# dotchen/LAV

Hardware: AMD Instinct MI355X
Metric: frames/s full agent fwd (32k-pt LiDAR + 3 cams) (higher is better)
Workload: dtype f32 (convolution contractions on the matrix cores with f32 accumulate at the error of an fp32 dot product, DESIGN 4.3: the layers on the split-operand kernel - BEV backbone, heads, crop stems, the brake net's mid-size layers - and ERFNet's persistent runs of pairs as two power-of-two-scaled fp16 pie

## Files before the change

### include/lav_amd.h

```cpp
#ifndef LAV_AMD_H
#define LAV_AMD_H

#include <stddef.h>
#include <stdint.h>

#ifdef __cplusplus
extern "C" {
#endif

#define LAV_ABI_VERSION 40

#define LAV_OK 0
#define LAV_EINVAL (-1)
#define LAV_EHIP (-2)
#define LAV_EWORKSPACE (-3)

int lav_abi_version(void);
const char *lav_last_error(void);
int lav_device_count(void);

int lav_profile_enable(int slots);
int lav_profile_reset(void);
int lav_profile_read(const char *kernel, double *total_ms, int *launches);

typedef struct lav_grid {
    float min_x, max_x, min_y, max_y;
    float ppm;
    int nx, ny;
} lav_grid;

typedef struct lav_pointnet {
    const float *w1, *b1, *w2, *b2;
    int num_input;
    int channels;
} lav_pointnet;

size_t lav_pillar_workspace_bytes(int batch, int max_points, const lav_grid *grid);
int lav_pillar_workspace_init(void *workspace, size_t workspace_bytes, void *stream);

int lav_pillar_scatter(const float *points, const int *h_num_points, int batch, int max_points, int D,
                       const lav_grid *grid, const lav_pointnet *net, float *canvas,
                       int *unique_coords, int *inverse, int *counts,
                       void *workspace, size_t workspace_bytes, void *stream);
// ... 180 lines not shown
int lav_upconv_pointwise_parts(int batch, int cin, int cout, int ih, int iw, int k, int pad, int out_pad);
int lav_upconv_pointwise(int batch, int cin, int cout, int ih, int iw, int k, int pad, int out_pad, const float *x, const float *w_packed,
                         const float *scale, const float *shift, int relu_pre, int out_c_total, int out_c_offset, float *y,
                         float *amax_out, void *stream);

size_t lav_conv1d_pair_packed_weight_floats(int channels);
int lav_conv1d_pair_pack_weights(int channels, const float *h_weight, float *h_packed);
size_t lav_conv1d_pair_chain_workspace_bytes(int batch, int h);
size_t lav_conv1d_pair_chain_lds_bytes(int channels, int w, int d_b_max);
int lav_conv1d_pair_chain(int batch, int channels, int h, int w, int npairs, const int *d_a, const int *d_b, const int *residual,
                          const int *relu_post, const float *x, const float *const *wa_packed, const float *const *bias_a,
                          const float *const *wb_packed, const float *const *bias_b, const float *const *scale,
                          const float *const *shift, float *const *out, void *workspace, size_t workspace_bytes, void *stream);
int lav_conv1d_pair_chain_f16(int batch, int channels, int h, int w, int npairs, const int *d_a, const int *d_b, const int *residual,
                              const int *relu_post, const float *x, const float *const *wa_packed, const float *const *bias_a,
                              const float *const *wb_packed, const float *const *bias_b, const float *const *scale,
                              const float *const *shift, float *const *out, void *workspace, size_t workspace_bytes, void *stream);
int lav_conv1d_pair_chain_region(int row_offset, int clean_rows);
int lav_conv1d_pair_chain_status(const void *workspace, int *h_timeouts_launches2, void *stream);
size_t lav_conv1d_pair_lds_bytes(int channels, int w, int d_b);
size_t lav_conv3x3_run_f16_workspace_bytes(int channels, int h, int w, int nlayers);
size_t lav_conv3x3_run_f16_lds_bytes(int channels, int h, int w);
size_t lav_conv3x3_run_f16_weight_bytes(int channels);
int lav_conv3x3_run_f16_amax_count(int channels, int h, int w);
long lav_conv_f16_weights_offset(const lav_conv *c);
int lav_conv3x3_run_f16(int channels, int h, int w, int nlayers, const float *x, const void *const *w_f16, const float *const *scale,
                        const float *const *shift, float *out, const float *amax_in, int amax_in_count, float *amax_out, void *workspace,
                        size_t workspace_bytes, void *stream);
int lav_conv3x3_run_f16_status(const void *workspace, int *h_timeouts_launches2, void *stream);
size_t lav_conv3x3_tile_f16_lds_bytes(int channels, int h, int w, int nlayers);
int lav_conv3x3_tile_f16_amax_count(int channels, int h, int w, int nlayers);
int lav_conv3x3_tile_f16(int channels, int h, int w, int nlayers, const float *x, const void *const *w_f16, const float *const *scale,
                         const float *const *shift, float *out, const float *amax_in, int amax_in_count, float *amax_out, void *stream);
int lav_conv1d_pair(int batch, int channels, int h, int w, int d_a, int d_b, const float *x, const float *wa_packed,
                    const float *bias_a, const float *wb_packed, const float *bias_b, const float *scale, const float *shift,
                    const float *residual, int relu_post, float *y, void *stream);

int lav_pool_affine(const float *x, int batch, int channels, int h, int w, const float *scale, const float *shift, int relu,
                    float *y, int out_c_total, int out_c_offset, void *stream);

int lav_pair_train_supported(int channels, int width);
size_t lav_pair_train_workspace_bytes(int batch, int channels, int h);
int lav_pair_train_forward(const float *x, const float *wa, const float *ba, const float *wb, const float *bb, int batch, int channels,
                           int h, int w, int dil, float *t, float *z, void *stream);
int lav_pair_train_backward(const float *x, const float *t, const float *dz, const float *wa, const float *wb, int batch, int channels,
                            int h, int w, int dil, float *dt, float *dx, float *dwa, float *dba, float *dwb, float *dbb, void *workspace,
                            size_t workspace_bytes, void *stream);

size_t lav_seg_xent_workspace_bytes(void);
int lav_seg_xent_forward(const float *logits, const long long *labels, int batch, int classes, long plane, float *loss, float *dlogits,
                         void *workspace, size_t workspace_bytes, void *stream);

int lav_seg_xent_up_forward(const float *logits, const void *labels, int label_bytes, int batch, int classes, int h, int w, int scale,
                            float *loss, float *dlogits, void *workspace, size_t workspace_bytes, void *stream);

typedef struct lav_camera_f64 {
    double l2w[16];
    double w2c[16];
    double K[9];
} lav_camera_f64;

int lav_paint_frames(const float *lidar, const int *offsets, int frames, int total, int lidar_dim, const float *sem, int ncam,
                     int sem_c, int h, int w, const lav_camera_f64 *h_cams, float *painted, int *uvz, void *stream);

int lav_image_u8_to_f32(const unsigned char *img, int n, int h, int w, int c_src, int reverse, float *out, void *stream);

// ... 59 lines not shown
```

### lav_amd/_lib.py

```python
from __future__ import annotations

import ctypes as C
import os

HERE = os.path.dirname(os.path.abspath(__file__))
LIB_PATH = os.environ.get("LAV_AMD_LIB") or os.path.join(HERE, "liblav_amd.so")

ABI_VERSION = 40
MAX_CAM = 4
MAX_CAM_F64 = 8


class Grid(C.Structure):
    _fields_ = [("min_x", C.c_float), ("max_x", C.c_float), ("min_y", C.c_float), ("max_y", C.c_float),
                ("ppm", C.c_float), ("nx", C.c_int), ("ny", C.c_int)]


class PointNet(C.Structure):
    _fields_ = [("w1", C.c_void_p), ("b1", C.c_void_p), ("w2", C.c_void_p), ("b2", C.c_void_p),
                ("num_input", C.c_int), ("channels", C.c_int)]


class Camera(C.Structure):
    _fields_ = [("K", C.c_float * 9), ("l2w", C.c_float * 16), ("w2c", C.c_float * 16)]


class CameraF64(C.Structure):
    _fields_ = [("l2w", C.c_double * 16), ("w2c", C.c_double * 16), ("K", C.c_double * 9)]


class Conv(C.Structure):
    _fields_ = [(n, C.c_int) for n in (
        "batch", "in_c_total", "in_c_offset", "cin", "h", "w", "cout", "kh", "kw", "stride", "pad_h", "pad_w",
        "dil_h", "dil_w", "transposed", "out_pad", "out_c_total", "out_c_offset", "relu_pre", "relu_post", "sigmoid", "target_cus")] + [("pad_value", C.c_float), ("precision", C.c_int)]


CONV_F32, CONV_BF16X6, CONV_F16X3 = 1, 2, 3


_P, _I, _Z, _F = C.c_void_p, C.c_int, C.c_size_t, C.c_float
SIGNATURES = {
# ... 28 lines not shown
    "lav_conv_pack_map_ints": (_Z, [C.POINTER(Conv)]),
    "lav_conv_pack_map": (_I, [C.POINTER(Conv), _P]),
    "lav_conv_repack": (_I, [C.POINTER(Conv), _P, _P, _P, _P]),
    "lav_conv_repack_scratch": (_I, [C.POINTER(Conv), _P, _P, _P, _P, _Z, _P]),
    "lav_bn_fold": (_I, [_P, _P, _P, _P, C.c_double, _I, _P, _P, _P]),
    "lav_conv_wgrad_workspace_bytes": (_Z, [_I, _I, _I, _I, _I, _I, _I]),
    "lav_conv_wgrad": (_I, [_P, _P, _I, _I, _I, _I, _I, _I, _I, _P, _P, _Z, _P]),
    "lav_conv_wgrad_amax": (_I, [_P, _P, _I, _I, _I, _I, _I, _I, _I, _P, _P, _Z, _P, _I, _P, _I, _P]),
    "lav_absmax_parts": (_I, [_P, C.c_long, _P, _P]),
    "lav_conv_tile_info": (_I, [C.POINTER(Conv), C.POINTER(_I)]),
    "lav_conv_workspace_bytes": (_Z, [C.POINTER(Conv)]),
    "lav_conv2d": (_I, [C.POINTER(Conv), _P, _P, _P, _P, _P, _P, _P, _P, _Z, _P]),
    "lav_conv_amax_count": (_I, [C.POINTER(Conv)]),
    "lav_conv2d_amax": (_I, [C.POINTER(Conv), _P, _P, _P, _P, _P, _P, _P, _P, _Z, _P, _I, _P, _P]),
    "lav_deconv_grouped": (_I, [_I, _I, _I, _I, _I, C.POINTER(_I), _I, _I, _I, _I, _P, _P, _P, _I, _P, _P]),
    "lav_crop_rotate": (_I, [_P, _I, _I, _I, _I, _P, _P, _I, _F, _I, _F, _F, _P, _P]),
    "lav_crop_rotate_indexed": (_I, [_P, _I, _P, _I, _I, _I, _P, _P, _I, _F, _I, _F, _F, _P, _P]),
    "lav_crop_rotate_backward": (_I, [_P, _I, _P, _I, _I, _I, _P, _P, _I, _F, _I, _F, _F, _P, _P]),
    "lav_pillar_decorate": (_I, [_P, C.POINTER(_I), _I, _I, _I, C.POINTER(Grid), _P, _P, _P, _P, _P, _P, _Z, _P]),
    "lav_scatter_max": (_I, [_P, _P, _I, _I, _I, _P, _P, _P]),
    "lav_scatter_max_backward": (_I, [_P, _P, _I, _I, _I, _P, _P]),
    "lav_conv1d_pair_packed_weight_floats": (_Z, [_I]),
    "lav_conv1d_pair_pack_weights": (_I, [_I, _P, _P]),
    "lav_upconv_pointwise_packed_floats": (_Z, [_I, _I, _I]),
    "lav_upconv_pointwise_pack": (_I, [_I, _I, _I, _P, _P]),
    "lav_upconv_pointwise_parts": (_I, [_I] * 8),
    "lav_upconv_pointwise": (_I, [_I] * 8 + [_P, _P, _P, _P, _I, _I, _I, _P, _P, _P]),
    "lav_conv1d_pair_chain_workspace_bytes": (_Z, [_I, _I]),
    "lav_conv1d_pair_chain_region": (_I, [_I, _I]),
    "lav_conv1d_pair_chain_lds_bytes": (_Z, [_I, _I, _I]),
    "lav_conv1d_pair_chain": (_I, [_I, _I, _I, _I, _I, C.POINTER(_I), C.POINTER(_I), C.POINTER(_I), C.POINTER(_I), _P] + [C.POINTER(_P)] * 7 + [_P, _Z, _P]),
    "lav_conv1d_pair_chain_f16": (_I, [_I, _I, _I, _I, _I, C.POINTER(_I), C.POINTER(_I), C.POINTER(_I), C.POINTER(_I), _P] + [C.POINTER(_P)] * 7 + [_P, _Z, _P]),
    "lav_conv1d_pair_chain_status": (_I, [_P, C.POINTER(_I), _P]),
    "lav_conv1d_pair_lds_bytes": (_Z, [_I, _I, _I]),
    "lav_conv3x3_run_f16_workspace_bytes": (_Z, [_I, _I, _I, _I]),
    "lav_conv3x3_run_f16_lds_bytes": (_Z, [_I, _I, _I]),
    "lav_conv3x3_run_f16_weight_bytes": (_Z, [_I]),
    "lav_conv3x3_run_f16_amax_count": (_I, [_I, _I, _I]),
    "lav_conv_f16_weights_offset": (C.c_long, [C.POINTER(Conv)]),
    "lav_conv3x3_run_f16": (_I, [_I, _I, _I, _I, _P, C.POINTER(_P), C.POINTER(_P), C.POINTER(_P), _P, _P, _I, _P, _P, _Z, _P]),
    "lav_conv3x3_run_f16_status": (_I, [_P, C.POINTER(_I), _P]),
    "lav_conv3x3_tile_f16_lds_bytes": (_Z, [_I, _I, _I, _I]),
    "lav_conv3x3_tile_f16_amax_count": (_I, [_I, _I, _I, _I]),
    "lav_conv3x3_tile_f16": (_I, [_I, _I, _I, _I, _P, C.POINTER(_P), C.POINTER(_P), C.POINTER(_P), _P, _P, _I, _P, _P]),
    "lav_conv1d_pair": (_I, [_I, _I, _I, _I, _I, _I, _P, _P, _P, _P, _P, _P, _P, _P, _I, _P, _P]),
    "lav_gru_seq_forward": (_I, [_P, _I, _P, _P, _P, _I, _I, _I, _P, _P, _P]),
    "lav_gru_seq_backward_workspace_bytes": (_Z, [_I, _I]),
    "lav_gru_seq_backward": (_I, [_P, _P, _P, _P, _P, _I, _I, _I, _P, _P, _P, _P, _Z, _P]),
    "lav_bn_train_workspace_bytes": (_Z, [_I]),
    "lav_bn_train_forward_mask": (_I, [_P, _P, _P, _P, _I, _I, C.c_long, _P, _P, C.c_double, _I, _P, _P, _P, _P, _P, _Z, _P]),
    "lav_bn_train_backward_mask": (_I, [_P, _P, _P, _P, _I, _I, C.c_long, _P, _P, _P, _I, _P, _P, _P, _P, _P, _P, _Z, _P]),
    "lav_pair_train_supported": (_I, [_I, _I]),
    "lav_pair_train_workspace_bytes": (_Z, [_I, _I, _I]),
    "lav_pair_train_forward": (_I, [_P, _P, _P, _P, _P, _I, _I, _I, _I, _I, _P, _P, _P]),
    "lav_pair_train_backward": (_I, [_P, _P, _P, _P, _P, _I, _I, _I, _I, _I, _P, _P, _P, _P, _P, _P, _P, _Z, _P]),
    "lav_seg_xent_workspace_bytes": (_Z, []),
    "lav_seg_xent_forward": (_I, [_P, _P, _I, _I, C.c_long, _P, _P, _P, _Z, _P]),
    "lav_seg_xent_up_forward": (_I, [_P, _P, _I, _I, _I, _I, _I, _I, _P, _P, _P, _Z, _P]),
    "lav_attn_train_workspace_bytes": (_Z, [_I, _I, _I, _I]),
    "lav_attn_train_forward": (_I, [_P, _I, _I, _I, _I, _P, _P, _P, _P, C.c_float, _P, _P, _P, _P, _P, _P]),
    "lav_attn_train_backward": (_I, [_P, _I, _I, _I, _I, _P, _P, _P, _P, C.c_float, _P, _P, _P, _P, _P, _P, _P, _P, _P, _Z, _P]),
    "lav_bn_train_forward": (_I, [_P, _P, _P, _I, _I, C.c_long, _P, _P, C.c_double, _I, _I, _P, _P, _P, _P, _Z, _P]),
    "lav_bn_train_backward": (_I, [_P, _P, _P, _I, _I, C.c_long, _P, _P, _P, _I, _I, _P, _P, _P, _P, _P, _Z, _P]),
    "lav_bn_train_amax_count": (_I, [_I, _I, C.c_long]),
    "lav_bn_train_forward_amax": (_I, [_P, _P, _P, _I, _I, C.c_long, _P, _P, C.c_double, _I, _I, _P, _P, _P, _P, _P, _Z, _P]),
    "lav_bn_train_backward_amax": (_I, [_P, _P, _P, _I, _I, C.c_long, _P, _P, _P, _I, _I, _P, _P, _P, _P, _P, _P, _Z, _P]),
# ... 66 lines not shown
```

### lav_amd/build.py

```python
from __future__ import annotations

import os
import subprocess
import sys
import time

HERE = os.path.dirname(os.path.abspath(__file__))
REPO = os.path.dirname(HERE)
CSRC = os.path.join(HERE, "csrc")
LIB = os.path.join(HERE, "liblav_amd.so")
SOURCES = ["misc.hip", "pillar.hip", "paint.hip", "paint_frames.hip", "gru.hip", "gru_seq.hip", "conv.hip", "conv_f16.hip", "conv_pair.hip", "conv_run.hip", "conv_tile.hip", "deconv.hip", "crop.hip", "frame.hip", "attn.hip", "bn_train.hip", "conv_wgrad.hip", "upconv.hip", "conv_pair_train.hip", "augment.hip", "bev_stack.hip", "debug_view.hip", "log_view.hip", "eval_metrics.hip", "eval_camera.hip", "eval_plans.hip"]
EXTRA_FLAGS = {"pillar.hip": ["-ffp-contract=off"], "paint.hip": ["-ffp-contract=off"], "paint_frames.hip": ["-ffp-contract=off"], "crop.hip": ["-ffp-contract=off"],
               "frame.hip": ["-ffp-contract=off"], "augment.hip": ["-ffp-contract=off"], "bev_stack.hip": ["-ffp-contract=off"],
               "debug_view.hip": ["-ffp-contract=off", "-fhip-fp32-correctly-rounded-divide-sqrt"],
               "log_view.hip": ["-ffp-contract=off"],
               "eval_metrics.hip": ["-ffp-contract=off"],
               "eval_plans.hip": ["-ffp-contract=off"]}
FLAGS = ["--offload-arch=gfx950", "-O3", "-std=c++17", "-fPIC", "-Wall", "-Wno-unused-function", "-fno-slp-vectorize",
         "-I", os.path.join(REPO, "include"), "-I", CSRC]


def _hipcc() -> str:
    for c in (os.environ.get("HIPCC"), "/opt/rocm/bin/hipcc", "hipcc"):
        if c and (os.path.isabs(c) and os.path.exists(c) or not os.path.isabs(c)):
            return c
    raise RuntimeError("hipcc not found")


def needs_build() -> bool:
    if not os.path.exists(LIB):
        return True
    t = os.path.getmtime(LIB)
    deps = [os.path.join(CSRC, f) for f in os.listdir(CSRC)] + [os.path.join(REPO, "include", "lav_amd.h")]
    return any(os.path.getmtime(d) > t for d in deps)


def build(force: bool = False, verbose: bool = True) -> str:
    if not force and not needs_build():
        return LIB
    objs = []
    procs = []
    os.makedirs(os.path.join(HERE, "build"), exist_ok=True)
    t0 = time.time()
    for s in SOURCES:
# ... 22 lines not shown
```

### lav_amd/erfnet.py

```python
from __future__ import annotations

import os

import torch
import torch.nn as nn
import torch.nn.functional as F

from . import ops
from .ops import Conv1dPair, Conv1dPairChain, ConvLayer, GroupedDeconv, infer_precision

_USE_PAIRS = os.environ.get("LAV_ERFNET_PAIRS", "1") != "0"


def _affine(bn, sl):
    s = (bn.weight.detach().double() / torch.sqrt(bn.running_var.detach().double() + bn.eps))
    t = bn.bias.detach().double() - bn.running_mean.detach().double() * s
    return s[sl].float()[None, :, None, None].contiguous(), t[sl].float()[None, :, None, None].contiguous()


class DownsamplerBlock(nn.Module):
    def __init__(self, cin, cout):
        super().__init__()
        self.conv = nn.Conv2d(cin, cout - cin, 3, stride=2, padding=1, bias=True)
        self.pool = nn.MaxPool2d(2, stride=2)
        self.bn = nn.BatchNorm2d(cout, eps=1e-3)

    def forward(self, x):
        return F.relu(self.bn(torch.cat([self.conv(x), self.pool(x)], 1)))

    def engine(self, device, input_affine=None):
        from . import ops
        nconv = self.conv.out_channels
        cout = self.bn.num_features
        w, b, pad = self.conv.weight.detach(), self.conv.bias.detach(), 0.0
        s_in, t_in = (1.0, 0.0) if input_affine is None else input_affine
        if input_affine is not None:
            if not s_in > 0:
                raise RuntimeError("input_affine needs a positive scale")
            b = (b.double() + t_in * w.double().sum(dim=(1, 2, 3))).float()
            w = (w.double() * s_in).float()
            pad = -t_in / s_in
        sl = slice(0, nconv)
# ... 34 lines not shown
        if self.dropout.p != 0:
            y = self.dropout(y)
        return F.relu(y + x)

    def engine(self, device):
        a = ConvLayer.from_module(self.conv3x1_1, relu_post=True, device=device)
        b = ConvLayer.from_module(self.conv1x3_1, self.bn1, relu_post=True, device=device)
        c = ConvLayer.from_module(self.conv3x1_2, relu_post=True, device=device)
        d = ConvLayer.from_module(self.conv1x3_2, self.bn2, relu_post=True, device=device)
        p1 = Conv1dPair(self.conv3x1_1, self.conv1x3_1, self.bn1, device=device)
        p2 = Conv1dPair(self.conv3x1_2, self.conv1x3_2, self.bn2, device=device)

        def run(x):
            if _USE_PAIRS and p1.supported(x) and p2.supported(x):
                return p2(p1(x), residual=x)
            return d(c(b(a(x))), residual=x)
        run.pairs = (p1, p2)
        return run


def _chain_blocks(stages):
    out, run = [], []

    def flush():
        if not run:
            return
        blocks = list(run)
        run.clear()
        if len(blocks) == 1 or not _USE_PAIRS:
            out.extend(blocks)
            return
        pairs = [p for b in blocks for p in b.pairs]
        chain = Conv1dPairChain(pairs, [i % 2 == 1 for i in range(len(pairs))])

        def go(x):
            if chain.supported(x):
                return chain(x)
            for b in blocks:
                x = b(x)
            return x
        go.chain = chain
        out.append(go)

    for st in stages:
        if getattr(st, "pairs", None) is not None and (not run or run[-1].pairs[0].ch == st.pairs[0].ch):
            run.append(st)
        else:
            flush()
            if getattr(st, "pairs", None) is not None:
                run.append(st)
            else:
                out.append(st)
    flush()
    return out


class UpsamplerBlock(nn.Module):
    def __init__(self, cin, cout):
        super().__init__()
        self.conv = nn.ConvTranspose2d(cin, cout, 3, stride=2, padding=1, output_padding=1, bias=True)
        self.bn = nn.BatchNorm2d(cout, eps=1e-3)

    def forward(self, x):
        return F.relu(self.bn(self.conv(x)))

    def engine(self, device):
        return ConvLayer.from_module(self.conv, self.bn, relu_post=True, device=device)


class Encoder(nn.Module):
    def __init__(self, num_classes):
        super().__init__()
        self.initial_block = DownsamplerBlock(3, 16)
        blocks = [DownsamplerBlock(16, 64)] + [non_bottleneck_1d(64, 0.03, 1) for _ in range(5)] + [DownsamplerBlock(64, 128)]
# ... 14 lines not shown
        self.layers = nn.ModuleList([UpsamplerBlock(128, 64), non_bottleneck_1d(64, 0, 1), non_bottleneck_1d(64, 0, 1),
                                     UpsamplerBlock(64, 16), non_bottleneck_1d(16, 0, 1), non_bottleneck_1d(16, 0, 1)])
        self.output_conv = nn.ConvTranspose2d(16, num_classes, 2, stride=2)

    def forward(self, x):
        for layer in self.layers:
            x = layer(x)
        return self.output_conv(x)


class ERFNet(nn.Module):
    def __init__(self, num_classes):
        super().__init__()
        self.encoder = Encoder(num_classes)
        self.decoder = Decoder(num_classes)
        object.__setattr__(self, "_eng", None)

    def _drop(self):
        object.__setattr__(self, "_eng", None)

    def _apply(self, fn, *a, **k):
        self._drop()
        return super()._apply(fn, *a, **k)

    def train(self, mode: bool = True):
        self._drop()
        return super().train(mode)

    def _load_from_state_dict(self, *a, **k):
        self._drop()
        return super()._load_from_state_dict(*a, **k)

    def _engine(self, device, input_affine=None, softmax=False):
        key = (device, input_affine, softmax, infer_precision())
        if self._eng is None or self._eng[0] != key:
            stages = [self.encoder.initial_block.engine(device, input_affine)]
            stages += [m.engine(device) for m in self.encoder.layers]
            stages += [m.engine(device) for m in self.decoder.layers]
            stages = _chain_blocks(stages)
            stages.append(GroupedDeconv([self.decoder.output_conv], softmax=softmax, device=device))
            object.__setattr__(self, "_eng", (key, stages))
        return self._eng[1]

    def forward(self, x, input_affine=None, softmax=False):
        if self.training:
            if input_affine is not None:
                x = x * input_affine[0] + input_affine[1]
            y = self.decoder(self.encoder(x))
            return torch.softmax(y, dim=1) if softmax else y
        if not x.is_cuda:
            raise RuntimeError("ERFNet: eval-mode forward needs a tensor in HBM - lav_amd has no CPU path "
                               "(CPU evaluation for tests and baselines: oracle/camera.py)")
        shared = os.environ.get("LAV_CHAIN_SHARED_CLEAN", "1") != "0"
        cap, off, first = ops.pair_chain_capacity(x.device), 0, True
        for stage in self._engine(x.device, input_affine, softmax):
            chain = getattr(stage, "chain", None)
            rows = x.shape[0] * x.shape[2]
            if shared and chain is not None and chain.supported(x) and off + rows <= cap:
                with ops.pair_chain_region(off, cap if first else 0):
                    x = stage(x)
                off, first = off + rows, False
            else:
                if chain is not None:
                    shared = False
                x = stage(x)
        return x
```

### lav_amd/ops.py

```python
from __future__ import annotations

import ctypes as C
import os as _os
import threading as _threading
from typing import Optional, Sequence

import numpy as np
import torch

from . import _lib
from ._lib import Camera, Conv, Grid, PointNet, check

_workspaces: dict = {}


def _stream() -> int:
    return torch.cuda.current_stream().cuda_stream


def _ptr(t: Optional[torch.Tensor]) -> Optional[int]:
    return None if t is None else t.data_ptr()


def _f32c(t: torch.Tensor, name: str) -> torch.Tensor:
# ... 1029 lines not shown


class Conv1dPairChain:

    def __init__(self, pairs, residual):
        if len(pairs) != len(residual) or not pairs or residual[0]:
            raise RuntimeError("Conv1dPairChain: one residual flag per pair, the first pair without")
        if any(p.ch != pairs[0].ch or p.scale is None for p in pairs):
            raise RuntimeError("Conv1dPairChain: pairs of one channel count, each with its BatchNorm affine")
        self.pairs, self.residual = list(pairs), [int(bool(r)) for r in residual]
        self._bufs = {}
        self.f16 = infer_precision() == _lib.CONV_F16X3 and _os.environ.get("LAV_ERFNET_F16", "1") != "0"

    def supported(self, x: torch.Tensor) -> bool:
        lib = _lib.load()
        B, ch, h, w = x.shape
        p0 = self.pairs[0]
        lds = lib.lav_conv1d_pair_chain_lds_bytes(p0.ch, w, max(p.db for p in self.pairs))
        return (_os.environ.get("LAV_CONV_PRECISION", "bf16x6") not in ("f32", "fp32") and _os.environ.get("LAV_ERFNET_CHAIN", "1") != "0"
                and len(self.pairs) <= 16 and all(p.supported(x) for p in self.pairs)
                and B * h <= _cu_count(x.device) * (2 if (lds <= 76 * 1024 and not (ch >= 64 and (ch // 16) % 2 == 0)) else 1)
                and lds <= 152 * 1024)

    def __call__(self, x: torch.Tensor) -> torch.Tensor:
        lib = _lib.load()
        x = _f32c(x, "x")
        B, ch, h, w = x.shape
        n = len(self.pairs)
        key = (B, h, w, x.device, _stream())
        bufs = self._bufs.get(key)
        if bufs is None:
            bufs = self._bufs[key] = [torch.empty_like(x) for _ in range(n - 1)]
        out = bufs + [torch.empty_like(x)]
        ws = _workspace("pair_chain", max(lib.lav_conv1d_pair_chain_workspace_bytes(B, h), lib.lav_conv1d_pair_chain_workspace_bytes(pair_chain_capacity(x.device), 1)), x.device)
        ia = lambda vals: (C.c_int * n)(*vals)
        pa = lambda ts: (C.c_void_p * n)(*[t.data_ptr() for t in ts])
        ps = self.pairs
        check((lib.lav_conv1d_pair_chain_f16 if self.f16 else lib.lav_conv1d_pair_chain)(B, ch, h, w, n, ia([p.da for p in ps]), ia([p.db for p in ps]), ia(self.residual),
                                        ia([int(p.relu_post) for p in ps]), _ptr(x), pa([p.wa for p in ps]), pa([p.ba for p in ps]),
                                        pa([p.wb for p in ps]), pa([p.bb for p in ps]), pa([p.scale for p in ps]), pa([p.shift for p in ps]),
                                        pa(out), _ptr(ws), ws.numel(), _stream()), "lav_conv1d_pair_chain")
        return out[-1]

    def timeouts(self, x_like: torch.Tensor) -> int:
        return pair_chain_status(x_like.device)[0]


def pair_chain_capacity(device) -> int:
    return 4 * _cu_count(device)


class pair_chain_region:

    def __init__(self, row_offset: int, clean_rows: int):
        self.args = (int(row_offset), int(clean_rows))

    def __enter__(self):
        check(_lib.load().lav_conv1d_pair_chain_region(*self.args), "lav_conv1d_pair_chain_region")
        return self

    def __exit__(self, *exc):
        check(_lib.load().lav_conv1d_pair_chain_region(0, -1), "lav_conv1d_pair_chain_region")
        return False


def pair_chain_status(device, stream=None):
    st = stream if stream is not None else torch.cuda.current_stream()
    device = torch.device(device)
    if device.index is None:
        device = torch.device("cuda", torch.cuda.current_device())
    ws = _workspaces.get(("pair_chain", device, st.cuda_stream))
    if ws is None:
        return (0, 0)
    v = (C.c_int * 2)()
    check(_lib.load().lav_conv1d_pair_chain_status(_ptr(ws), v, st.cuda_stream), "lav_conv1d_pair_chain_status")
    return (int(v[0]), int(v[1]))


def bev_run_stages():
    v = _os.environ.get("LAV_BEV_RUN", BEV_RUN_DEFAULT).strip().lower()
    if v in ("0", "", "off", "none"):
        return frozenset()
    if v in ("1", "on", "all"):
        return frozenset(("s1", "s2", "s3"))
    return frozenset(s for s in v.split(",") if s in ("s1", "s2", "s3"))


BEV_RUN_DEFAULT = "s2,s3"


class ConvRun:

    def __init__(self, layers):
        lib = _lib.load()
        layers = list(layers)
        l0 = layers[0]
        for l in layers:
            d = l.desc
            if not (d.precision == _lib.CONV_F16X3 and (d.kh, d.kw, d.stride, d.pad_h, d.pad_w, d.dil_h, d.dil_w) == (3, 3, 1, 1, 1, 1, 1)
                    and not d.transposed and l.cin == l.cout == l0.cin and l.in_c_total == l.cin and l.out_c_total == l.cout
                    and l.bias is None and l.scale is not None and d.relu_pre and not d.relu_post and not d.sigmoid and d.pad_value == 0.0):
                raise RuntimeError("ConvRun: layers must be identical conv3x3 / ReLU / BatchNorm layers packed for LAV_CONV_F16X3")
        self.layers, self.ch = layers, l0.cin
        probe = Conv.from_buffer_copy(l0.desc)
        probe.h, probe.w = 64, 64
        self._woff = int(lib.lav_conv_f16_weights_offset(C.byref(probe)))
        if self._woff < 0 or len(layers) > 8:
            raise RuntimeError("ConvRun: at most 8 layers with fp16 packed weights")
        n = len(layers)
# ... 324 lines not shown
```

Measured before the change: 541.0.

## Add spatially tiled fused non-bottleneck-1d kernel for ERFNet dilation-1 blocks

Adds a new kernel that runs one or two whole ERFNet non-bottleneck-1d blocks (four 1D convolution pairs with BN, ReLU and residual) inside a single workgroup per spatial tile. Activations stay in LDS as split fp16 pieces with a halo, and the next layer's weights are prefetched into registers while the current layer runs. The goal is to avoid the global round-trips and row-wise chain scheduling of the existing pair-chain path. By default it is enabled only for the 16-channel, two-block stage, at the cost of recomputing halo regions and a large LDS footprint.

```diff
diff --git a/include/lav_amd.h b/include/lav_amd.h
--- a/include/lav_amd.h
+++ b/include/lav_amd.h
@@ -8,7 +8,7 @@
 extern "C" {
 #endif
 
-#define LAV_ABI_VERSION 40
+#define LAV_ABI_VERSION 41
 
 #define LAV_OK 0
 #define LAV_EINVAL (-1)
@@ -255,6 +255,10 @@
 int lav_conv3x3_tile_f16_amax_count(int channels, int h, int w, int nlayers);
 int lav_conv3x3_tile_f16(int channels, int h, int w, int nlayers, const float *x, const void *const *w_f16, const float *const *scale,
                          const float *const *shift, float *out, const float *amax_in, int amax_in_count, float *amax_out, void *stream);
+size_t lav_nb1d_tile_f16_lds_bytes(int channels, int h, int w, int nblocks);
+int lav_nb1d_tile_f16(int batch, int channels, int h, int w, int nblocks, const float *x, const float *const *wa_packed,
+                      const float *const *bias_a, const float *const *wb_packed, const float *const *bias_b, const float *const *scale,
+                      const float *const *shift, float *out, void *count_workspace, void *stream);
 int lav_conv1d_pair(int batch, int channels, int h, int w, int d_a, int d_b, const float *x, const float *wa_packed,
                     const float *bias_a, const float *wb_packed, const float *bias_b, const float *scale, const float *shift,
                     const float *residual, int relu_post, float *y, void *stream);
diff --git a/lav_amd/_lib.py b/lav_amd/_lib.py
--- a/lav_amd/_lib.py
+++ b/lav_amd/_lib.py
@@ -6,7 +6,7 @@
 HERE = os.path.dirname(os.path.abspath(__file__))
 LIB_PATH = os.environ.get("LAV_AMD_LIB") or os.path.join(HERE, "liblav_amd.so")
 
-ABI_VERSION = 40
+ABI_VERSION = 41
 MAX_CAM = 4
 MAX_CAM_F64 = 8
 
@@ -101,6 +101,8 @@
     "lav_conv1d_pair_chain": (_I, [_I, _I, _I, _I, _I, C.POINTER(_I), C.POINTER(_I), C.POINTER(_I), C.POINTER(_I), _P] + [C.POINTER(_P)] * 7 + [_P, _Z, _P]),
     "lav_conv1d_pair_chain_f16": (_I, [_I, _I, _I, _I, _I, C.POINTER(_I), C.POINTER(_I), C.POINTER(_I), C.POINTER(_I), _P] + [C.POINTER(_P)] * 7 + [_P, _Z, _P]),
     "lav_conv1d_pair_chain_status": (_I, [_P, C.POINTER(_I), _P]),
+    "lav_nb1d_tile_f16_lds_bytes": (_Z, [_I, _I, _I, _I]),
+    "lav_nb1d_tile_f16": (_I, [_I, _I, _I, _I, _I, _P] + [C.POINTER(_P)] * 6 + [_P, _P, _P]),
     "lav_conv1d_pair_lds_bytes": (_Z, [_I, _I, _I]),
     "lav_conv3x3_run_f16_workspace_bytes": (_Z, [_I, _I, _I, _I]),
     "lav_conv3x3_run_f16_lds_bytes": (_Z, [_I, _I, _I]),
diff --git a/lav_amd/build.py b/lav_amd/build.py
--- a/lav_amd/build.py
+++ b/lav_amd/build.py
@@ -9,7 +9,7 @@
 REPO = os.path.dirname(HERE)
 CSRC = os.path.join(HERE, "csrc")
 LIB = os.path.join(HERE, "liblav_amd.so")
-SOURCES = ["misc.hip", "pillar.hip", "paint.hip", "paint_frames.hip", "gru.hip", "gru_seq.hip", "conv.hip", "conv_f16.hip", "conv_pair.hip", "conv_run.hip", "conv_tile.hip", "deconv.hip", "crop.hip", "frame.hip", "attn.hip", "bn_train.hip", "conv_wgrad.hip", "upconv.hip", "conv_pair_train.hip", "augment.hip", "bev_stack.hip", "debug_view.hip", "log_view.hip", "eval_metrics.hip", "eval_camera.hip", "eval_plans.hip"]
+SOURCES = ["misc.hip", "pillar.hip", "paint.hip", "paint_frames.hip", "gru.hip", "gru_seq.hip", "conv.hip", "conv_f16.hip", "conv_pair.hip", "conv_pair_tile.hip", "conv_run.hip", "conv_tile.hip", "deconv.hip", "crop.hip", "frame.hip", "attn.hip", "bn_train.hip", "conv_wgrad.hip", "upconv.hip", "conv_pair_train.hip", "augment.hip", "bev_stack.hip", "debug_view.hip", "log_view.hip", "eval_metrics.hip", "eval_camera.hip", "eval_plans.hip"]
 EXTRA_FLAGS = {"pillar.hip": ["-ffp-contract=off"], "paint.hip": ["-ffp-contract=off"], "paint_frames.hip": ["-ffp-contract=off"], "crop.hip": ["-ffp-contract=off"],
                "frame.hip": ["-ffp-contract=off"], "augment.hip": ["-ffp-contract=off"], "bev_stack.hip": ["-ffp-contract=off"],
                "debug_view.hip": ["-ffp-contract=off", "-fhip-fp32-correctly-rounded-divide-sqrt"],
diff --git a/lav_amd/csrc/conv_pair_tile.hip b/lav_amd/csrc/conv_pair_tile.hip
--- /dev/null
+++ b/lav_amd/csrc/conv_pair_tile.hip
@@ -0,0 +1,424 @@
+#include <cstdlib>
+#include <cstring>
+
+#include "common.hpp"
+#include "split_arith.hpp"
+
+namespace {
+using namespace lav;
+
+constexpr int NBT_MAX_NB = 2, NBT_MAX_PAIRS = 2 * NBT_MAX_NB;
+
+struct NbTileArgs {
+    const float *x;
+    float *out;
+    const unsigned char *wA[NBT_MAX_PAIRS], *wB[NBT_MAX_PAIRS];
+    const float *tA[NBT_MAX_PAIRS], *tB[NBT_MAX_PAIRS];
+    const float *bA[NBT_MAX_PAIRS], *bB[NBT_MAX_PAIRS], *scale[NBT_MAX_PAIRS], *shift[NBT_MAX_PAIRS];
+    int *count;
+    int H, W, tiles_x, tiles_y;
+};
+
+template <int C>
+struct NbGeo {
+    static constexpr int NCH = C / 16, CBLK = (C + 31) / 32, NGRP = 8 / CBLK, NG8 = C / 8;
+    static constexpr int NPART = C >= 64 ? 2 : 1;
+    static constexpr int NGV = C >= 32 ? 4 : C / 8;
+    static constexpr int WB = 3 * NCH * CBLK * 2 * 1024;
+    static constexpr int NPF = (WB / 16 + 511) / 512;
+};
+
+template <int C>
+__device__ __forceinline__ void nbt_w_fetch(const unsigned char *w, u32x4 (&pf)[NbGeo<C>::NPF]) {
+#pragma unroll
+    for (int k = 0; k < NbGeo<C>::NPF; ++k) {
+        const int u = threadIdx.x + 512 * k;
+        pf[k] = *reinterpret_cast<const u32x4 *>(w + min(u, NbGeo<C>::WB / 16 - 1) * 16);
+    }
+}
+template <int C>
+__device__ __forceinline__ void nbt_w_store(unsigned char *wl, const u32x4 (&pf)[NbGeo<C>::NPF]) {
+#pragma unroll
+    for (int k = 0; k < NbGeo<C>::NPF; ++k) {
+        const int u = threadIdx.x + 512 * k;
+        if (u < NbGeo<C>::WB / 16) *reinterpret_cast<u32x4 *>(wl + u * 16) = pf[k];
+    }
+}
+
+template <int C, int NA, int MAXJ, bool VERT, int IW, int NPI>
+__device__ __forceinline__ void nbt_mma(const unsigned char *in, const int (&base)[MAXJ], int half, const unsigned char *wl, f32x16 (&tot)[MAXJ]) {
+    using G = NbGeo<C>;
+    constexpr int PIECE = G::NG8 * NPI * 16, CPP = G::NCH / G::NPART;
+#pragma unroll
+    for (int part = 0; part < G::NPART; ++part) {
+        f32x16 acc[NA];
+#pragma unroll
+        for (int j = 0; j < NA; ++j)
+#pragma unroll
+            for (int r = 0; r < 16; ++r) acc[j][r] = 0.f;
+#pragma unroll
+        for (int i = 0; i < CPP; ++i) {
+            const int ch = part * CPP + i;
+            const unsigned char *bin = in + (ch * 2 + half) * NPI * 16;
+#pragma unroll
+            for (int t = 0; t < 3; ++t) {
+                const int toff = (VERT ? t * IW : t) * 16;
+                u32x4 b[NA][2], wf[2];
+                wf[0] = *reinterpret_cast<const u32x4 *>(wl + (t * G::NCH + ch) * G::CBLK * 2048);
+                wf[1] = *reinterpret_cast<const u32x4 *>(wl + (t * G::NCH + ch) * G::CBLK * 2048 + 1024);
+#pragma unroll
+                for (int j = 0; j < NA; ++j) {
+                    b[j][0] = *reinterpret_cast<const u32x4 *>(bin + toff + base[j]);
+                    b[j][1] = *reinterpret_cast<const u32x4 *>(bin + PIECE + toff + base[j]);
+                }
+#pragma unroll
+                for (int k = 0; k < 3; ++k)
+#pragma unroll
+                    for (int j = 0; j < NA; ++j)
+                        acc[j] = __builtin_amdgcn_mfma_f32_32x32x16_f16(__builtin_bit_cast(f16x8, wf[F16X3_A[k]]), __builtin_bit_cast(f16x8, b[j][F16X3_B[k]]),
+                                                                        acc[j], 0, 0, 0);
+            }
+        }
+#pragma unroll
+        for (int j = 0; j < NA; ++j) {
+            if (part == 0) tot[j] = acc[j];
+            else
+#pragma unroll
+                for (int r = 0; r < 16; ++r) tot[j][r] += acc[j][r];
+        }
+    }
+}
+
+enum { NBT_MID = 0,
+       NBT_PAIR = 1,
+       NBT_BLOCK = 2,
+       NBT_LAST = 3 };
+
+struct NbtScale { float s, m; };
+
+template <int C, int TH, int TW, int IH, int IW, bool VERT, int KIND, bool RES_LDS>
+__device__ __forceinline__ NbtScale nbt_layer(const NbTileArgs &a, int n, int ty0, int tx0, const unsigned char *in, unsigned char *outb, float *res, int iy0, int ix0,
+                                              NbtScale sc, float sw, float l1, float bmax, const float *epi, float *s_wmax, unsigned char *wlds,
+                                              const unsigned char *w_next) {
+    using G = NbGeo<C>;
+    constexpr int OH = VERT ? IH - 2 : IH, OW = VERT ? IW : IW - 2, NP = OH * OW, NPI = IH * IW;
+    constexpr int NBLK = (NP + 31) / 32, MAXJ = (NBLK + G::NGRP - 1) / G::NGRP;
+    const int tid = threadIdx.x, lane = tid & 63, l31 = lane & 31, half = lane >> 5;
+    const int wid = __builtin_amdgcn_readfirstlane(tid >> 6);
+    const int cbw = wid % G::CBLK, grp = wid / G::CBLK;
+    const int H = a.H, W = a.W;
+    const long plane = (long)H * W;
+    const int oy0 = VERT ? iy0 + 1 : iy0, ox0 = VERT ? ix0 : ix0 + 1;
+
+    int qu[MAXJ], base[MAXJ];
+#pragma unroll
+    for (int j = 0; j < MAXJ; ++j) {
+        qu[j] = (grp + G::NGRP * j) * 32 + l31;
+        const int q = min(qu[j], NP - 1);
+        base[j] = ((q / OW) * IW + (q % OW)) * 16;
+    }
+    const int nact = (NBLK - grp + G::NGRP - 1) / G::NGRP;
+
+    float rin[(KIND >= NBT_BLOCK && !RES_LDS) ? MAXJ : 1][16];
+    if constexpr (KIND >= NBT_BLOCK && !RES_LDS) {
+#pragma unroll
+        for (int j = 0; j < MAXJ; ++j) {
+            const int q = min(qu[j], NP - 1);
+            const int gy = oy0 + q / OW, gx = ox0 + q % OW;
+            const bool ok = j < nact && gy >= 0 && gy < H && gx >= 0 && gx < W;
+            const float *xr = a.x + (long)n * C * plane + (long)min(max(gy, 0), H - 1) * W + min(max(gx, 0), W - 1);
+#pragma unroll
+            for (int r = 0; r < 16; ++r) {
+                const int co = min(cbw * 32 + (r & 3) + 8 * (r >> 2) + 4 * half, C - 1);
+                rin[j][r] = ok ? xr[co * plane] : 0.f;
+            }
+        }
+    }
+
+    u32x4 pf[G::NPF];
+    if constexpr (KIND != NBT_LAST) nbt_w_fetch<C>(w_next, pf);
+    f32x16 acc[MAXJ];
+#pragma unroll
+    for (int j = 0; j < MAXJ; ++j)
+#pragma unroll
+        for (int r = 0; r < 16; ++r) acc[j][r] = 0.f;
+    const unsigned char *wl = wlds + cbw * 2048 + lane * 16;
+    if (nact == MAXJ) nbt_mma<C, MAXJ, MAXJ, VERT, IW, NPI>(in, base, half, wl, acc);
+    else if constexpr (MAXJ > 1) nbt_mma<C, MAXJ - 1, MAXJ, VERT, IW, NPI>(in, base, half, wl, acc);
+    if constexpr (KIND == NBT_MID) __syncthreads();
+
+    NbtScale so;
+    float f_in, inv_out = 0.f;
+    if constexpr (KIND == NBT_MID) {
+        so.m = fminf(fmaf(sc.m, l1, bmax), 3.0e38f);
+        so.s = f16_scale_of(so.m);
+        inv_out = 1.f / so.s;
+    }
+    f_in = sc.s * sw;
+    float lm = 0.f;
+    bool inmap[MAXJ];
+#pragma unroll
+    for (int j = 0; j < MAXJ; ++j) {
+        const int q = min(qu[j], NP - 1);
+        const int qy = q / OW, qx = q % OW, gy = oy0 + qy, gx = ox0 + qx;
+        inmap[j] = j < nact && qu[j] < NP && gy >= 0 && gy < H && gx >= 0 && gx < W;
+        float *yo = a.out + (long)n * C * plane + (long)gy * W + gx;
+#pragma unroll
+        for (int r = 0; r < 16; ++r) {
+            if ((r >> 2) >= G::NGV) { acc[j][r] = 0.f; continue; }
+            const int co = cbw * 32 + (r & 3) + 8 * (r >> 2) + 4 * half;
+            float vv;
+            if constexpr (KIND == NBT_MID) {
+                vv = fmaf(acc[j][r], f_in, epi[co]);
+                vv = vv > 0.f ? vv : 0.f;
+            } else {
+                vv = fmaf(fmaf(acc[j][r], f_in, epi[C + co]), epi[2 * C + co], epi[3 * C + co]);
+                if constexpr (KIND >= NBT_BLOCK) {
+                    if constexpr (RES_LDS) vv += inmap[j] ? res[co * (TH * TW) + q] : 0.f;
+                    else vv += rin[j][r];
+                }
+                vv = vv > 0.f ? vv : 0.f;
+            }
+            vv = inmap[j] ? vv : 0.f;
+            if constexpr (KIND == NBT_LAST) {
+                if (inmap[j]) yo[co * plane] = vv;
+            } else {
+                acc[j][r] = vv;
+                lm = fmaxf(lm, finite_abs(vv));
+            }
+            if constexpr (KIND == NBT_BLOCK) {
+                const int ry = qy - 2, rx = qx - 2;
+                if (j < nact && qu[j] < NP && ry >= 0 && ry < TH && rx >= 0 && rx < TW) res[co * (TH * TW) + ry * TW + rx] = vv;
+            }
+        }
+    }
+    if constexpr (KIND == NBT_LAST) return NbtScale{0.f, 0.f};
+    if constexpr (KIND != NBT_MID) {
+        lm = wave_finite_absmax(lm);
+        if (lane == 0) s_wmax[wid] = lm;
+        __syncthreads();
+        float m = 0.f;
+#pragma unroll
+        for (int i = 0; i < 8; ++i) m = fmaxf(m, s_wmax[i]);
+        so.m = m;
+        so.s = f16_scale_of(m);
+        inv_out = 1.f / so.s;
+    }
+#pragma unroll
+    for (int j = 0; j < MAXJ; ++j) {
+        if (j < nact && qu[j] < NP) {
+#pragma unroll
+            for (int g = 0; g < G::NGV; ++g) {
+                unsigned p00, p01, p10, p11;
+                split2h_pair(acc[j][4 * g] * inv_out, acc[j][4 * g + 1] * inv_out, p00, p10);
+                split2h_pair(acc[j][4 * g + 2] * inv_out, acc[j][4 * g + 3] * inv_out, p01, p11);
+                unsigned char *d = outb + ((cbw * 4 + g) * NP + qu[j]) * 16 + half * 8;
+                *reinterpret_cast<u32x2 *>(d) = u32x2{p00, p01};
+                lds_store_fence();
+                *reinterpret_cast<u32x2 *>(d + G::NG8 * NP * 16) = u32x2{p10, p11};
+                lds_store_fence();
+            }
+        }
+    }
+    nbt_w_store<C>(wlds, pf);
+    __syncthreads();
+    return so;
+}
+
+template <int C, int TH, int TW, int NB>
+struct NbTileLds {
+    static constexpr int RH = TH + 4 * NB, RW = TW + 4 * NB;
+    static constexpr int BUF_A = 2 * (C / 8) * RH * RW * 16, BUF_B = 2 * (C / 8) * (RH - 2) * RW * 16;
+    static constexpr int RES = NB > 1 ? TH * TW * C * 4 : 0, EPI = 2 * NB * 4 * C * 4, WB = NbGeo<C>::WB;
+    static constexpr int TOTAL = BUF_A + BUF_B + RES + WB + EPI + 64;
+};
+
+template <int C, int TH, int TW, int IH, int IW, bool LAST, bool RES_LDS>
+__device__ __forceinline__ NbtScale nbt_block(const NbTileArgs &a, int n, int ty0, int tx0, unsigned char *bufA, unsigned char *bufB, float *res, int iy0, int ix0,
+                                              NbtScale sc, int p0, const float (&bmax)[NBT_MAX_PAIRS], const float (&tl)[NBT_MAX_PAIRS][3], const float *s_epi, float *s_wmax,
+                                              unsigned char *wr, const unsigned char *w_after) {
+    const float *e0 = s_epi + p0 * 4 * C, *e1 = e0 + 4 * C;
+    NbtScale s = nbt_layer<C, TH, TW, IH, IW, true, NBT_MID, false>(a, n, ty0, tx0, bufA, bufB, res, iy0, ix0, sc, tl[p0][0], tl[p0][1], bmax[p0], e0, s_wmax, wr,
+                                                                    a.wB[p0]);
+    s = nbt_layer<C, TH, TW, IH - 2, IW, false, NBT_PAIR, false>(a, n, ty0, tx0, bufB, bufA, res, iy0 + 1, ix0, s, tl[p0][2], 0.f, 0.f, e0, s_wmax, wr, a.wA[p0 + 1]);
+    s = nbt_layer<C, TH, TW, IH - 2, IW - 2, true, NBT_MID, false>(a, n, ty0, tx0, bufA, bufB, res, iy0 + 1, ix0 + 1, s, tl[p0 + 1][0], tl[p0 + 1][1], bmax[p0 + 1], e1,
+                                                                   s_wmax, wr, a.wB[p0 + 1]);
+    return nbt_layer<C, TH, TW, IH - 4, IW - 2, false, LAST ? NBT_LAST : NBT_BLOCK, RES_LDS>(a, n, ty0, tx0, bufB, bufA, res, iy0 + 2, ix0 + 1, s, tl[p0 + 1][2], 0.f, 0.f,
+                                                                                            e1, s_wmax, wr, w_after);
+}
+
+template <int C, int TH, int TW, int NB>
+__global__ __launch_bounds__(512) void k_nb1d_tile_f16(NbTileArgs a) {
+    using G = NbGeo<C>;
+    using L = NbTileLds<C, TH, TW, NB>;
+    extern __shared__ __attribute__((aligned(16))) unsigned char smem[];
+    constexpr int RH = L::RH, RW = L::RW, NPA = RH * RW, HALO = 2 * NB;
+    unsigned char *bufA = smem, *bufB = smem + L::BUF_A;
+    float *res = reinterpret_cast<float *>(smem + L::BUF_A + L::BUF_B);
+    unsigned char *wr = smem + L::BUF_A + L::BUF_B + L::RES;
+    float *s_epi = reinterpret_cast<float *>(smem + L::BUF_A + L::BUF_B + L::RES + L::WB);
+    float *s_wmax = s_epi + 2 * NB * 4 * C;
+    const int tid = threadIdx.x, lane = tid & 63;
+    const int wid = __builtin_amdgcn_readfirstlane(tid >> 6);
+    const int H = a.H, W = a.W;
+    const long plane = (long)H * W;
+    const int tiles = a.tiles_x * a.tiles_y;
+    const int n = blockIdx.x / tiles, t_ = blockIdx.x - n * tiles;
+    const int ty0 = (t_ / a.tiles_x) * TH, tx0 = (t_ % a.tiles_x) * TW;
+    if (blockIdx.x == 0 && tid == 0 && a.count) atomicAdd(a.count, 1);
+
+    NbtScale sc;
+    float bmax[NBT_MAX_PAIRS], tails[NBT_MAX_PAIRS][3];
+    {
+        constexpr int NTASK = NPA * G::NG8, NTK = (NTASK + 511) / 512, NEPI = 2 * NB * 4 * C;
+        static_assert(NEPI <= 512, "one epilogue value per thread");
+        float v[NTK][8];
+        bool ok[NTK];
+#pragma unroll
+        for (int u = 0; u < NTK; ++u) {
+            const int task = min(tid + u * 512, NTASK - 1);
+            const int g = task / NPA, p = task - g * NPA;
+            const int gy = ty0 - HALO + p / RW, gx = tx0 - HALO + p % RW;
+            ok[u] = gy >= 0 && gy < H && gx >= 0 && gx < W;
+            const float *sp = a.x + ((long)n * C + g * 8) * plane + (long)min(max(gy, 0), H - 1) * W + min(max(gx, 0), W - 1);
+#pragma unroll
+            for (int c = 0; c < 8; ++c) v[u][c] = sp[c * plane];
+        }
+        u32x4 pf[G::NPF];
+        nbt_w_fetch<C>(a.wA[0], pf);
+        float ev, braw[NBT_MAX_PAIRS];
+        {
+            const int i = min(tid, NEPI - 1), p = i / (4 * C), k = (i / C) & 3, c = i % C;
+            ev = (k == 0 ? a.bA[p] : k == 1 ? a.bB[p] : k == 2 ? a.scale[p] : a.shift[p])[c];
+        }
+#pragma unroll
+        for (int p = 0; p < NBT_MAX_PAIRS; ++p) {
+            braw[p] = a.bA[p][min(lane, C - 1)];
+            tails[p][0] = a.tA[p][0]; tails[p][1] = a.tA[p][1]; tails[p][2] = a.tB[p][0];
+        }
+        float lm = 0.f;
+#pragma unroll
+        for (int u = 0; u < NTK; ++u)
+#pragma unroll
+            for (int c = 0; c < 8; ++c) {
+                v[u][c] = ok[u] ? v[u][c] : 0.f;
+                lm = fmaxf(lm, finite_abs(v[u][c]));
+            }
+        nbt_w_store<C>(wr, pf);
+        if (tid < NEPI) s_epi[tid] = ev;
+#pragma unroll
+        for (int p = 0; p < NBT_MAX_PAIRS; ++p) bmax[p] = wave_finite_absmax(finite_abs(braw[p]));
+        lm = wave_finite_absmax(lm);
+        if (lane == 0) s_wmax[wid] = lm;
+        __syncthreads();
+        float m = 0.f;
+#pragma unroll
+        for (int i = 0; i < 8; ++i) m = fmaxf(m, s_wmax[i]);
+        sc.m = m;
+        sc.s = f16_scale_of(m);
+        const float inv = 1.f / sc.s;
+#pragma unroll
+        for (int u = 0; u < NTK; ++u) {
+            const int task = tid + u * 512;
+            if (task < NTASK) {
+                u32x4 q0, q1;
+#pragma unroll
+                for (int e = 0; e < 4; ++e) {
+                    unsigned p0, p1;
+                    split2h_pair(v[u][2 * e] * inv, v[u][2 * e + 1] * inv, p0, p1);
+                    q0[e] = p0; q1[e] = p1;
+                }
+                *reinterpret_cast<u32x4 *>(bufA + task * 16) = q0;
+                *reinterpret_cast<u32x4 *>(bufA + L::BUF_A / 2 + task * 16) = q1;
+            }
+        }
+    }
+    __syncthreads();
+
+    if constexpr (NB == 1) {
+        nbt_block<C, TH, TW, RH, RW, true, false>(a, n, ty0, tx0, bufA, bufB, res, ty0 - 2, tx0 - 2, sc, 0, bmax, tails, s_epi, s_wmax, wr, nullptr);
+    } else {
+        sc = nbt_block<C, TH, TW, RH, RW, false, false>(a, n, ty0, tx0, bufA, bufB, res, ty0 - 4, tx0 - 4, sc, 0, bmax, tails, s_epi, s_wmax, wr, a.wA[2]);
+        nbt_block<C, TH, TW, RH - 4, RW - 4, true, true>(a, n, ty0, tx0, bufA, bufB, res, ty0 - 2, tx0 - 2, sc, 2, bmax, tails, s_epi, s_wmax, wr, nullptr);
+    }
+}
+
+struct NbTileConfig { int th, tw, tiles_x, tiles_y; size_t lds; };
+
+bool nbt_wide() {
+    static const bool v = [] { const char *e = getenv("LAV_ERFNET_TILE_SHAPE"); return e && !strcmp(e, "wide"); }();
+    return v;
+}
+
+template <int C, int TH, int TW, int NB>
+constexpr size_t nbt_lds() { return (size_t)NbTileLds<C, TH, TW, NB>::TOTAL; }
+
+bool nbt_config(int channels, int h, int w, int nblocks, NbTileConfig &c) {
+    if ((channels != 16 && channels != 64) || nblocks < 1 || nblocks > NBT_MAX_NB || h < 1 || w < 1 || h > 32768 || w > 32768) return false;
+    const bool wide = nbt_wide();
+    if (channels == 64) {
+        if (nblocks != 1) return false;
+        c.th = 8; c.tw = 8;
+        c.lds = nbt_lds<64, 8, 8, 1>();
+    } else {
+        c.th = 16; c.tw = wide ? 32 : 16;
+        c.lds = wide ? (nblocks == 1 ? nbt_lds<16, 16, 32, 1>() : nbt_lds<16, 16, 32, 2>()) : (nblocks == 1 ? nbt_lds<16, 16, 16, 1>() : nbt_lds<16, 16, 16, 2>());
+    }
+    c.tiles_x = (w + c.tw - 1) / c.tw;
+    c.tiles_y = (h + c.th - 1) / c.th;
+    return c.lds <= 160 * 1024;
+}
+
+template <int C, int TH, int TW, int NB>
+int nbt_launch(const NbTileArgs &a, const NbTileConfig &c, int batch, hipStream_t st) {
+    static_assert(NbTileLds<C, TH, TW, NB>::TOTAL <= 160 * 1024, "LDS of a workgroup");
+    static bool attr = false;
+    if (!attr) {
+        LAV_HIP(hipFuncSetAttribute(reinterpret_cast<const void *>(&k_nb1d_tile_f16<C, TH, TW, NB>), hipFuncAttributeMaxDynamicSharedMemorySize, 160 * 1024));
+        attr = true;
+    }
+    hipLaunchKernelGGL((k_nb1d_tile_f16<C, TH, TW, NB>), dim3(batch * c.tiles_x * c.tiles_y), dim3(512), c.lds, st, a);
+    return LAV_OK;
+}
+}
+
+extern "C" size_t lav_conv1d_pair_packed_weight_floats(int channels);
+
+extern "C" size_t lav_nb1d_tile_f16_lds_bytes(int channels, int h, int w, int nblocks) {
+    NbTileConfig c;
+    return nbt_config(channels, h, w, nblocks, c) ? c.lds : 0;
+}
+
+extern "C" int lav_nb1d_tile_f16(int batch, int channels, int h, int w, int nblocks, const float *x, const float *const *wa_packed, const float *const *bias_a,
+                                 const float *const *wb_packed, const float *const *bias_b, const float *const *scale, const float *const *shift, float *out,
+                                 void *count_workspace, void *stream) {
+    NbTileConfig c;
+    LAV_REQUIRE(nbt_config(channels, h, w, nblocks, c), "lav_nb1d_tile_f16: %d blocks of %d channels on %d x %d are not served (lav_nb1d_tile_f16_lds_bytes returns 0)",
+                nblocks, channels, h, w);
+    LAV_REQUIRE(batch >= 1 && (long)batch * c.tiles_x * c.tiles_y <= (1l << 20), "lav_nb1d_tile_f16: batch %d: too many tiles", batch);
+    LAV_REQUIRE(x && wa_packed && bias_a && wb_packed && bias_b && scale && shift && out && x != out, "lav_nb1d_tile_f16: null argument (or out == x)");
+    const size_t f16_floats = (size_t)3 * (channels / 16) * ((channels + 31) / 32) * 2 * 1024 / 4;
+    const size_t sec = lav_conv1d_pair_packed_weight_floats(channels) - 4 - f16_floats;
+    NbTileArgs a;
+    for (int i = 0; i < NBT_MAX_PAIRS; ++i) {
+        const int j = i < 2 * nblocks ? i : 2 * nblocks - 1;
+        LAV_REQUIRE(wa_packed[j] && bias_a[j] && wb_packed[j] && bias_b[j] && scale[j] && shift[j], "lav_nb1d_tile_f16: null argument of pair %d", j);
+        a.wA[i] = reinterpret_cast<const unsigned char *>(wa_packed[j] + sec);
+        a.wB[i] = reinterpret_cast<const unsigned char *>(wb_packed[j] + sec);
+        a.tA[i] = wa_packed[j] + sec + f16_floats;
+        a.tB[i] = wb_packed[j] + sec + f16_floats;
+        a.bA[i] = bias_a[j]; a.bB[i] = bias_b[j]; a.scale[i] = scale[j]; a.shift[i] = shift[j];
+    }
+    a.x = x; a.out = out; a.count = count_workspace ? static_cast<int *>(count_workspace) + 1 : nullptr;
+    a.H = h; a.W = w; a.tiles_x = c.tiles_x; a.tiles_y = c.tiles_y;
+    hipStream_t st = static_cast<hipStream_t>(stream);
+    const int tok = timer_begin("nb1d_tile", st);
+    int rc;
+    if (channels == 64) rc = nbt_launch<64, 8, 8, 1>(a, c, batch, st);
+    else if (c.tw == 32) rc = nblocks == 1 ? nbt_launch<16, 16, 32, 1>(a, c, batch, st) : nbt_launch<16, 16, 32, 2>(a, c, batch, st);
+    else rc = nblocks == 1 ? nbt_launch<16, 16, 16, 1>(a, c, batch, st) : nbt_launch<16, 16, 16, 2>(a, c, batch, st);
+    if (rc != LAV_OK) return rc;
+    timer_end(tok, st);
+    LAV_LAUNCH_CHECK();
+    return LAV_OK;
+}
diff --git a/lav_amd/erfnet.py b/lav_amd/erfnet.py
--- a/lav_amd/erfnet.py
+++ b/lav_amd/erfnet.py
@@ -7,7 +7,7 @@
 import torch.nn.functional as F
 
 from . import ops
-from .ops import Conv1dPair, Conv1dPairChain, ConvLayer, GroupedDeconv, infer_precision
+from .ops import Conv1dPair, Conv1dPairChain, ConvLayer, GroupedDeconv, Nb1dTileRun, infer_precision
 
 _USE_PAIRS = os.environ.get("LAV_ERFNET_PAIRS", "1") != "0"
 
@@ -108,14 +108,19 @@
             return
         pairs = [p for b in blocks for p in b.pairs]
         chain = Conv1dPairChain(pairs, [i % 2 == 1 for i in range(len(pairs))])
+        tile = None
+        if pairs[0].ch in (16, 64) and all(p.da == p.db == 1 for p in pairs) and ops.erfnet_tile_wants(pairs[0].ch, len(blocks)):
+            tile = Nb1dTileRun(pairs, [i % 2 == 1 for i in range(len(pairs))])
 
         def go(x):
+            if tile is not None and tile.takes(x):
+                return tile(x)
             if chain.supported(x):
                 return chain(x)
             for b in blocks:
                 x = b(x)
             return x
-        go.chain = chain
+        go.chain, go.tile = chain, tile
         out.append(go)
 
     for st in stages:
@@ -196,7 +201,7 @@
         return super()._load_from_state_dict(*a, **k)
 
     def _engine(self, device, input_affine=None, softmax=False):
-        key = (device, input_affine, softmax, infer_precision())
+        key = (device, input_affine, softmax, infer_precision(), ops.erfnet_tile_mode())
         if self._eng is None or self._eng[0] != key:
             stages = [self.encoder.initial_block.engine(device, input_affine)]
             stages += [m.engine(device) for m in self.encoder.layers]
@@ -218,6 +223,10 @@
         shared = os.environ.get("LAV_CHAIN_SHARED_CLEAN", "1") != "0"
         cap, off, first = ops.pair_chain_capacity(x.device), 0, True
         for stage in self._engine(x.device, input_affine, softmax):
+            tile = getattr(stage, "tile", None)
+            if tile is not None and tile.takes(x):
+                x = stage(x)
+                continue
             chain = getattr(stage, "chain", None)
             rows = x.shape[0] * x.shape[2]
             if shared and chain is not None and chain.supported(x) and off + rows <= cap:
diff --git a/lav_amd/ops.py b/lav_amd/ops.py
--- a/lav_amd/ops.py
+++ b/lav_amd/ops.py
@@ -1085,7 +1085,7 @@
         if bufs is None:
             bufs = self._bufs[key] = [torch.empty_like(x) for _ in range(n - 1)]
         out = bufs + [torch.empty_like(x)]
-        ws = _workspace("pair_chain", max(lib.lav_conv1d_pair_chain_workspace_bytes(B, h), lib.lav_conv1d_pair_chain_workspace_bytes(pair_chain_capacity(x.device), 1)), x.device)
+        ws = _pair_chain_workspace(B, h, x.device)
         ia = lambda vals: (C.c_int * n)(*vals)
         pa = lambda ts: (C.c_void_p * n)(*[t.data_ptr() for t in ts])
         ps = self.pairs
@@ -1097,6 +1097,11 @@
 
     def timeouts(self, x_like: torch.Tensor) -> int:
         return pair_chain_status(x_like.device)[0]
+
+
+def _pair_chain_workspace(B: int, h: int, device) -> torch.Tensor:
+    lib = _lib.load()
+    return _workspace("pair_chain", max(lib.lav_conv1d_pair_chain_workspace_bytes(B, h), lib.lav_conv1d_pair_chain_workspace_bytes(pair_chain_capacity(device), 1)), device)
 
 
 def pair_chain_capacity(device) -> int:
@@ -1128,6 +1133,68 @@
     v = (C.c_int * 2)()
     check(_lib.load().lav_conv1d_pair_chain_status(_ptr(ws), v, st.cuda_stream), "lav_conv1d_pair_chain_status")
     return (int(v[0]), int(v[1]))
+
+
+ERFNET_TILE_DEFAULT = "1"
+ERFNET_TILE_WON = frozenset({(16, 2)})
+NB1D_TILE_NB = {16: 2, 64: 1}
+
+
+def erfnet_tile_mode() -> str:
+    v = _os.environ.get("LAV_ERFNET_TILE", ERFNET_TILE_DEFAULT).strip().lower()
+    return "0" if v in ("0", "", "off", "none") else "all" if v == "all" else "1"
+
+
+def erfnet_tile_wants(ch: int, nblocks: int) -> bool:
+    mode = erfnet_tile_mode()
+    return mode == "all" or (mode == "1" and (ch, nblocks) in ERFNET_TILE_WON)
+
+
+class Nb1dTileRun:
+
+    def __init__(self, pairs, residual):
+        pairs = list(pairs)
+        if len(pairs) < 2 or len(pairs) % 2 or [int(bool(r)) for r in residual] != [i % 2 for i in range(len(pairs))]:
+            raise RuntimeError("Nb1dTileRun: two pairs per block, the second of each with the residual")
+        if any(p.ch != pairs[0].ch or p.scale is None or not p.relu_post for p in pairs):
+            raise RuntimeError("Nb1dTileRun: pairs of one channel count, each with its BatchNorm affine and ReLU")
+        self.pairs, self.ch, self.nblocks = pairs, pairs[0].ch, len(pairs) // 2
+        self.f16 = infer_precision() == _lib.CONV_F16X3 and _os.environ.get("LAV_ERFNET_F16", "1") != "0"
+        nb = int(_os.environ.get("LAV_ERFNET_TILE_NB", "0") or 0)
+        nb = nb if nb in (1, 2) else NB1D_TILE_NB.get(self.ch, 1)
+        self.cut = [nb] * (self.nblocks // nb) + ([self.nblocks % nb] if self.nblocks % nb else [])
+        self._bufs = {}
+
+    def takes(self, x: torch.Tensor) -> bool:
+        B, ch, h, w = x.shape
+        lib = _lib.load()
+        return (self.f16 and ch == self.ch and ch in (16, 64) and all(p.da == 1 and p.db == 1 for p in self.pairs)
+                and _os.environ.get("LAV_CONV_PRECISION", "bf16x6") not in ("f32", "fp32")
+                and all(lib.lav_nb1d_tile_f16_lds_bytes(ch, h, w, nb) > 0 for nb in set(self.cut)))
+
+    def __call__(self, x: torch.Tensor, out: Optional[torch.Tensor] = None) -> torch.Tensor:
+        lib = _lib.load()
+        x = _f32c(x, "x")
+        if out is not None and (out.shape != x.shape or out.dtype != torch.float32 or not out.is_contiguous() or out.data_ptr() == x.data_ptr()):
+            raise RuntimeError("Nb1dTileRun: out must be a contiguous float32 tensor of x's shape, and not x")
+        if not self.takes(x):
+            raise RuntimeError(f"Nb1dTileRun: input {tuple(x.shape)} is not served (lav_nb1d_tile_f16_lds_bytes, dilation 1, LAV_CONV_F16X3)")
+        B, ch, h, w = x.shape
+        key = (B, h, w, x.device, _stream())
+        bufs = self._bufs.get(key)
+        if bufs is None:
+            bufs = self._bufs[key] = [torch.empty_like(x) for _ in range(min(2, len(self.cut) - 1))]
+        ws = _pair_chain_workspace(B, h, x.device)
+        src, b0 = x, 0
+        for i, nb in enumerate(self.cut):
+            dst = (out if out is not None else torch.empty_like(x)) if i + 1 == len(self.cut) else bufs[i % 2]
+            ps = self.pairs[2 * b0: 2 * (b0 + nb)]
+            pa = lambda ts: (C.c_void_p * len(ps))(*[t.data_ptr() for t in ts])
+            check(lib.lav_nb1d_tile_f16(B, ch, h, w, nb, _ptr(src), pa([p.wa for p in ps]), pa([p.ba for p in ps]), pa([p.wb for p in ps]),
+                                        pa([p.bb for p in ps]), pa([p.scale for p in ps]), pa([p.shift for p in ps]), _ptr(dst),
+                                        _ptr(ws) if i == 0 else None, _stream()), "lav_nb1d_tile_f16")
+            src, b0 = dst, b0 + nb
+        return src
 
 
 def bev_run_stages():
```

After: 538.0. About the same (-0.6%).
